# 0xPARC/plonky2-aes

Hardware: AMD Instinct MI355X
Metric: proofs/sec (AES-GCM 1 KiB circuit) (higher is better)
Workload: dtype u64 (Goldilocks field)

## Files before the change

plonky2-aes_amd/csrc/kernels.h:

```cpp
#pragma once
#include <hip/hip_runtime.h>

#include "circuit.h"
#include "witness_schedule.h"
#include "gl.h"
#include "poseidon_fast.h"
#include "poseidon_gate.h"
#include "ecstep_gate.h"
#include "zk_prf.h"

namespace p2k {
using gl::E2;
using gl::u32;
using gl::u64;

static const u64 UNSET = ~0ull;

#ifndef P2_HASH_WAVES_PER_EU
#define P2_HASH_WAVES_PER_EU 5
#endif
#define P2_HASH_WAVES __attribute__((amdgpu_waves_per_eu(P2_HASH_WAVES_PER_EU, P2_HASH_WAVES_PER_EU)))

__global__ __launch_bounds__(256) P2_HASH_WAVES void k_hash_leaves(const u64* __restrict__ data, int cols, int active_cols, size_t col_stride,
                                                      size_t batch_stride, size_t num_leaves, u64* __restrict__ digests,
                                                      size_t dig_batch_stride) {
    if ((size_t)blockIdx.x * blockDim.x + threadIdx.x >= num_leaves) return;
    const u64* d = data + (size_t)blockIdx.y * batch_stride + ((size_t)blockIdx.x * blockDim.x + threadIdx.x);
    u64 st[12];
#pragma unroll
    for (int i = 0; i < 12; i++) st[i] = 0;
    if (cols <= 4) {
        u64* out = digests + (size_t)blockIdx.y * dig_batch_stride + ((size_t)blockIdx.x * blockDim.x + threadIdx.x) * 4;
        for (int c = 0; c < 4; c++) out[c] = (c < cols && c < active_cols) ? d[(size_t)c * col_stride] : 0;
        return;
    }
    for (int c0 = 0; c0 < cols; c0 += 8) {
#pragma unroll
        for (int k = 0; k < 8; k++) {
            int c = c0 + k;
            if (c < cols) st[k] = c < active_cols ? d[(size_t)k * col_stride] : 0;
        }
        d += 8 * col_stride;
        glf::sponge_permute(st, c0, cols, active_cols);
    }
    u64* out = digests + (size_t)blockIdx.y * dig_batch_stride + ((size_t)blockIdx.x * blockDim.x + threadIdx.x) * 4;
#pragma unroll
    for (int i = 0; i < 4; i++) out[i] = st[i];
}

__global__ __launch_bounds__(256) P2_HASH_WAVES void k_hash_fri_leaves(const u64* __restrict__ vals, size_t len, size_t batch_stride, int arity,
                                                          u64* __restrict__ digests, size_t dig_batch_stride) {
    size_t leaf = (size_t)blockIdx.x * blockDim.x + threadIdx.x;
    size_t num_leaves = len / arity;
    if (leaf >= num_leaves) return;
    const u64* v = vals + (size_t)blockIdx.y * batch_stride;
    u64 st[12];
#pragma unroll
    for (int i = 0; i < 12; i++) st[i] = 0;
    int width = 2 * arity;
    for (int e0 = 0; e0 < width; e0 += 8) {
#pragma unroll
        for (int k = 0; k < 8; k++) {
            int e = e0 + k;
            if (e < width) st[k] = v[(size_t)(e & 1) * len + leaf * arity + (e >> 1)];
        }
        glf::sponge_permute(st, e0, width, width);
    }
    u64* out = digests + (size_t)blockIdx.y * dig_batch_stride + leaf * 4;
#pragma unroll
    for (int i = 0; i < 4; i++) out[i] = st[i];
}

__global__ __launch_bounds__(256) P2_HASH_WAVES void k_merkle_level(const u64* __restrict__ child, u64* __restrict__ parent, size_t num_parents,
                                                       size_t batch_stride) {
    if ((size_t)blockIdx.x * blockDim.x + threadIdx.x >= num_parents) return;
    u64 st[12];
    {
        const u64* c = child + (size_t)blockIdx.y * batch_stride + 8 * ((size_t)blockIdx.x * blockDim.x + threadIdx.x);
#pragma unroll
        for (int k = 0; k < 8; k++) st[k] = c[k];
    }
#pragma unroll
    for (int k = 8; k < 12; k++) st[k] = 0;
    glf::two_to_one_permute(st);
    u64* o = parent + (size_t)blockIdx.y * batch_stride + 4 * ((size_t)blockIdx.x * blockDim.x + threadIdx.x);
#pragma unroll
    for (int k = 0; k < 4; k++) o[k] = st[k];
}

__global__ __launch_bounds__(256) P2_HASH_WAVES void k_merkle_top(u64* __restrict__ dig, size_t batch_stride, u32 bits, u32 first_level, u32 num_levels) {
    u64* base = dig + (size_t)blockIdx.y * batch_stride;
    u32 P = ((1u << bits) >> (first_level + 1)) / gridDim.x;
    for (u32 k = 0, l = first_level; k < num_levels; k++, l++, P >>= 1) {
        if (threadIdx.x < P) {
            const size_t off_c = 4 * (((size_t)2 << bits) - ((size_t)2 << (bits - l))), off_p = 4 * (((size_t)2 << bits) - ((size_t)2 << (bits - l - 1)));
            const size_t idx = (size_t)blockIdx.x * P + threadIdx.x;
            u64 st[12];
            {
                const u64* c = base + off_c + 8 * idx;
#pragma unroll
                for (int q = 0; q < 8; q++) st[q] = c[q];
            }
#pragma unroll
            for (int q = 8; q < 12; q++) st[q] = 0;
            glf::two_to_one_permute(st);
            u64* o = base + off_p + 4 * idx;
#pragma unroll
            for (int q = 0; q < 4; q++) o[q] = st[q];
        }
        __syncthreads();
    }
}
__global__ __launch_bounds__(256) void k_merkle_top_coop(u64* __restrict__ dig, size_t batch_stride, u32 bits, u32 first_level, u32 num_levels) {
    u64* base = dig + (size_t)blockIdx.y * batch_stride;
    u32 P = ((1u << bits) >> (first_level + 1)) / gridDim.x;
    const u32 g = threadIdx.x >> 4, i = threadIdx.x & 15;
    for (u32 k = 0, l = first_level; k < num_levels; k++, l++, P >>= 1) {
        const size_t off_c = 4 * (((size_t)2 << bits) - ((size_t)2 << (bits - l))), off_p = 4 * (((size_t)2 << bits) - ((size_t)2 << (bits - l - 1)));
        for (u32 first = 0; first < P; first += blockDim.x >> 4) {
            if (first + ((threadIdx.x >> 6) << 2) < P) {
                const u32 idx = first + g;
                const bool live = idx < P;
                const size_t node = (size_t)blockIdx.x * P + (live ? idx : 0);
                u64 w = (live && i < 8) ? base[off_c + 8 * node + i] : 0;
                w = glf::poseidon_coop(w, i);
                if (live && i < 4) base[off_p + 4 * node + i] = w;
            }
        }
        __syncthreads();
    }
}

__global__ void k_poseidon_states(u64* states, size_t n) {
    size_t i = (size_t)blockIdx.x * blockDim.x + threadIdx.x;
    if (i >= n) return;
    u64 st[12];
    for (int k = 0; k < 12; k++) st[k] = states[12 * i + k];
    glf::poseidon(st);
    for (int k = 0; k < 12; k++) states[12 * i + k] = st[k];
}

__global__ __launch_bounds__(256) P2_HASH_WAVES void k_partial_rounds(u64* states, size_t n) {
    size_t i = (size_t)blockIdx.x * blockDim.x + threadIdx.x;
    if (i >= n) return;
    u64 st[12];
    for (int k = 0; k < 12; k++) st[k] = states[12 * i + k];
    glf::partial_block(st);
    for (int k = 0; k < 12; k++) states[12 * i + k] = st[k];
}

__global__ __launch_bounds__(256) P2_HASH_WAVES void k_merged_middle(u64* states, size_t n) {
    size_t i = (size_t)blockIdx.x * blockDim.x + threadIdx.x;
    if (i >= n) return;
    u64 st[12];
    for (int k = 0; k < 12; k++) st[k] = states[12 * i + k];
    glf::merged_middle(st);
    for (int k = 0; k < 12; k++) states[12 * i + k] = st[k];
}

struct NttArgs {
    const u64* in;
    u64* out;
    const u64* tw;
    const u64* pre;
    const u64* pre_tw;
    const u64* post;
    u64 post_scalar;
    size_t in_col_stride, out_col_stride, in_batch_stride, out_batch_stride;
    int logn, log_nmax, cosets;
    int bitrev_in, bitrev_out;
    int in_coset_blocks;
    u32 block_of_coset[8];
};

__global__ __launch_bounds__(1024) void k_ntt_lds(NttArgs a) {
    extern __shared__ __align__(16) u64 lds[];
    const int logn = a.logn;
    const u32 n = 1u << logn;
    const u32 col = blockIdx.x / a.cosets, coset = blockIdx.x % a.cosets;
    const u32 blk = a.block_of_coset[coset];
    const u64* in = a.in + (size_t)blockIdx.y * a.in_batch_stride + (size_t)col * a.in_col_stride + (a.in_coset_blocks ? (size_t)blk * n : 0);
    u64* out = a.out + (size_t)blockIdx.y * a.out_batch_stride + (size_t)col * a.out_col_stride + (size_t)blk * n;
    const u64* pre = a.pre ? a.pre + (size_t)coset * n : nullptr;
    const u64* post = a.post ? a.post + (size_t)coset * n : nullptr;
    for (u32 i = threadIdx.x; i < n; i += blockDim.x) {
        u64 v = in[i];
        u32 dst = a.bitrev_in ? (__brev(i) >> (32 - logn)) : i;
        if (pre) v = gl::mul_nb(v, pre[dst]);
        lds[dst] = v;
    }
    __syncthreads();
    const int tw_shift = a.log_nmax - logn;
    int s = logn - 1;
    if (logn & 1) {
        const u32 h = 1u << s;
        for (u32 t = threadIdx.x; t < (n >> 1); t += blockDim.x) {
            u32 pos = t & (h - 1);
            u32 i = ((t >> s) << (s + 1)) | pos;
            u64 x = lds[i], y = lds[i + h];
            u64 w = a.tw[(size_t)(pos << (logn - 1 - s)) << tw_shift];
            lds[i] = gl::add(x, y);
            lds[i + h] = gl::mul_nb(gl::sub(x, y), w);
        }
        __syncthreads();
        s--;
    }
    for (; s >= 1; s -= 2) {
        const u32 h = 1u << s, q = h >> 1;
        for (u32 t = threadIdx.x; t < (n >> 2); t += blockDim.x) {
            u32 pos = t & (q - 1);
            u32 i = ((t >> (s - 1)) << (s + 1)) | pos;
            u64 a0 = lds[i], a1 = lds[i + q], a2 = lds[i + h], a3 = lds[i + h + q];
            u64 w0 = a.tw[(size_t)(pos << (logn - 1 - s)) << tw_shift];
            u64 w1 = a.tw[(size_t)((pos + q) << (logn - 1 - s)) << tw_shift];
            u64 b0 = gl::add(a0, a2), b2 = gl::mul_nb(gl::sub(a0, a2), w0);
            u64 b1 = gl::add(a1, a3), b3 = gl::mul_nb(gl::sub(a1, a3), w1);
            u64 w2 = a.tw[(size_t)(pos << (logn - s)) << tw_shift];
            lds[i] = gl::add(b0, b1);
            lds[i + q] = gl::mul_nb(gl::sub(b0, b1), w2);
            lds[i + h] = gl::add(b2, b3);
            lds[i + h + q] = gl::mul_nb(gl::sub(b2, b3), w2);
        }
        __syncthreads();
    }
    for (u32 i = threadIdx.x; i < n; i += blockDim.x) {
        u32 src = a.bitrev_out ? (__brev(i) >> (32 - logn)) : i;
        u64 v = lds[src];
        if (post)
            v = gl::mul_nb(v, post[i]);
        else if (a.post_scalar != 1)
            v = gl::mul_nb(v, a.post_scalar);
        out[i] = v;
    }
}

__device__ __forceinline__ u32 ntt_pad(u32 i) { return i + (i >> 4); }
struct NttLdsWalk {
    u32 a0, step;
    __device__ __forceinline__ NttLdsWalk(u32 base, u32 stride) : a0(8 * ntt_pad(base)), step(stride >= 16 ? 8 * (stride + (stride >> 4)) : 8 * stride) {}
    __device__ __forceinline__ u64& at(u64* lds, int r) const { return *(u64*)((char*)lds + (a0 + (u32)r * step)); }
};
__device__ __forceinline__ void ntt_r16_load_tw(u64* w, const u64* __restrict__ tw, u32 tp, int m, int tw_log, int nstages) {
#pragma unroll
    for (int A = 0; A < 4; A++) {
        if (A >= nstages) break;
        const int half = 8 >> A, base = 16 - 2 * half, sh = tw_log - (m + 4 - A);
        const u32 off0 = tp << (sh + 3), dj = 1u << (m + sh + 3);
#pragma unroll
        for (int j = 0; j < 8; j++)
            if (j < half) w[base + j] = *(const u64*)((const char*)tw + (off0 + (u32)j * dj));
    }
}
template <int A>
__device__ __forceinline__ void ntt_r16_stage(u64* x, const u64* w) {
    constexpr int half = 8 >> A, base = 16 - 2 * half;
#pragma unroll
    for (int r = 0; r < 16; r++) {
        if (r & half) continue;
        const u64 u = x[r], v = x[r + half];
        x[r] = gl::add(u, v);
        x[r + half] = gl::mul_nb(gl::sub(u, v), w[base + r % half]);
    }
}
template <int A>
__device__ __forceinline__ void ntt_r16_stage_m0(u64* x, const u64* w) {
    constexpr int half = 8 >> A, base = 16 - 2 * half;
#pragma unroll
    for (int r = 0; r < 16; r++) {
        if (r & half) continue;
        const u64 u = x[r], v = x[r + half];
        x[r] = gl::add(u, v);
        x[r + half] = (r % half) ? gl::mul_nb(gl::sub(u, v), w[base + r % half]) : gl::sub(u, v);
    }
}
__device__ __forceinline__ void wave_lds_sync() {
    __builtin_amdgcn_fence(__ATOMIC_RELEASE, "wavefront");
    __builtin_amdgcn_wave_barrier();
    __builtin_amdgcn_fence(__ATOMIC_ACQUIRE, "wavefront");
}
__device__ __forceinline__ u32 xcd_swizzle(u32 b, u32 grid) { return (grid & 7) ? b : (b & 7) * (grid >> 3) + (b >> 3); }
__device__ __forceinline__ void loads_issued() { asm volatile("" ::: "memory"); }
template <bool SPLIT>
__global__ __launch_bounds__(1024) void k_ntt_r16(NttArgs a) {
    extern __shared__ __align__(16) u64 lds[];
    const int logn = SPLIT ? a.logn - 1 : a.logn;
    const u32 n = 1u << logn, T = n >> 4, t = threadIdx.x;
    const u32 bid = xcd_swizzle(blockIdx.x, gridDim.x);
    const u32 unit = SPLIT ? bid >> 1 : bid, half = SPLIT ? (bid & 1) : 0;
    const u32 col = unit / a.cosets, coset = unit % a.cosets;
    const u32 blk = a.block_of_coset[coset];
    const size_t full = (size_t)1 << a.logn;
    const u64* in = a.in + (size_t)blockIdx.y * a.in_batch_stride + (size_t)col * a.in_col_stride + (a.in_coset_blocks ? (size_t)blk * full : 0);
    u64* out = a.out + (size_t)blockIdx.y * a.out_batch_stride + (size_t)col * a.out_col_stride + (size_t)blk * full + (size_t)half * n;
    const u64* pre = a.pre ? a.pre + (size_t)coset * full : nullptr;
    const u64* post = a.post ? a.post + (size_t)coset * full : nullptr;
    u64 x[16];
    u64 w[15];
    bool tw_in_flight = false;
    if (SPLIT) {
        if (pre) {
            const u64 S = pre[n];
            const u64* scale = half ? (a.pre_tw ? a.pre_tw + (size_t)coset * n : nullptr) : pre;
            if (!half || scale) {
                u64 uu[16], vv[16], sc[16];
#pragma unroll
                for (int k = 0; k < 16; k++) uu[k] = in[t + T * k];
#pragma unroll
                for (int k = 0; k < 16; k++) vv[k] = in[t + T * k + n];
#pragma unroll
                for (int k = 0; k < 8; k++) sc[k] = scale[t + T * k];
                loads_issued();
#pragma unroll
                for (int k = 0; k < 16; k++) {
                    if (k == 4) {
                        loads_issued();
#pragma unroll
                        for (int j = 8; j < 16; j++) sc[j] = scale[t + T * j];
                        loads_issued();
                    }
                    if (k == 12) {
                        loads_issued();
                        ntt_r16_load_tw(w, a.tw, t, logn - 4, a.log_nmax, 4);
                        loads_issued();
                    }
                    const u64 v = gl::mul_nb(vv[k], S);
                    x[k] = gl::mul_nb(half ? gl::sub(uu[k], v) : gl::add(uu[k], v), sc[k]);
                }
                tw_in_flight = true;
            } else {
#pragma unroll
                for (int k = 0; k < 16; k++) {
                    const u32 i = t + T * k;
                    const u64 u = in[i], v = gl::mul_nb(in[i + n], S);
                    x[k] = gl::mul_nb(gl::mul_nb(gl::sub(u, v), pre[i]), a.tw[(size_t)i << (a.log_nmax - a.logn)]);
                }
            }
        } else {
#pragma unroll
            for (int k = 0; k < 16; k++) {
                const u32 i = t + T * k;
                const u64 u = in[i], v = in[i + n];
                x[k] = half ? gl::mul_nb(gl::sub(u, v), a.tw[(size_t)i << (a.log_nmax - a.logn)]) : gl::add(u, v);
            }
        }
    } else if (a.bitrev_in) {
#pragma unroll
        for (int k = 0; k < 16; k++) {
            const u32 i = t + T * k, dst = __brev(i) >> (32 - logn);
            u64 v = in[i];
            if (pre) v = gl::mul_nb(v, pre[dst]);
            lds[ntt_pad(dst)] = v;
        }
        __syncthreads();
        {
            const NttLdsWalk w0(t, T);
#pragma unroll
            for (int k = 0; k < 16; k++) x[k] = w0.at(lds, k);
        }
    } else {
#pragma unroll
        for (int k = 0; k < 16; k++) x[k] = in[t + T * k];
        const int rem0 = (logn & 3) ? (logn & 3) : 4;
        if (pre) {
            u64 pv[16];
#pragma unroll
            for (int k = 0; k < 16; k++) pv[k] = pre[t + T * k];
            loads_issued();
#pragma unroll
            for (int k = 0; k < 16; k++) {
                if (k == 8) {
                    loads_issued();
                    ntt_r16_load_tw(w, a.tw, t, logn - 4, a.log_nmax, rem0);
                    loads_issued();
                }
                x[k] = gl::mul_nb(x[k], pv[k]);
            }
        } else {
            ntt_r16_load_tw(w, a.tw, t, logn - 4, a.log_nmax, rem0);
            loads_issued();
        }
        tw_in_flight = true;
    }
    if (SPLIT) {
        if (!tw_in_flight) ntt_r16_load_tw(w, a.tw, t, logn - 4, a.log_nmax, 4);
        ntt_r16_stage<0>(x, w);
        ntt_r16_stage<1>(x, w);
        ntt_r16_stage<2>(x, w);
        ntt_r16_stage<3>(x, w);
        int logN = logn - 4;
        const int rem = (logN & 3) ? (logN & 3) : 4;
        int m = logN - 4;
        u32 tp = t & ((1u << m) - 1);
        ntt_r16_load_tw(w, a.tw, tp, m, a.log_nmax, rem);
        {
            const NttLdsWalk wr(t, T);
#pragma unroll
            for (int r = 0; r < 16; r++) wr.at(lds, r) = x[r];
        }
        __syncthreads();
        u32 base_idx = ((t >> m) << logN) | tp, stride = 1u << m;
        {
            const NttLdsWalk rd(base_idx, stride);
#pragma unroll
            for (int r = 0; r < 16; r++) x[r] = rd.at(lds, r);
        }
        ntt_r16_stage<0>(x, w);
        if (rem >= 2) ntt_r16_stage<1>(x, w);
        if (rem >= 3) ntt_r16_stage<2>(x, w);
        if (rem >= 4) ntt_r16_stage<3>(x, w);
        for (logN -= rem; logN >= 4; logN -= 4) {
            m = logN - 4;
            tp = t & ((1u << m) - 1);
            ntt_r16_load_tw(w, a.tw, tp, m, a.log_nmax, 4);
            {
                const NttLdsWalk wr(base_idx, stride);
#pragma unroll
                for (int r = 0; r < 16; r++) wr.at(lds, r) = x[r];
            }
            wave_lds_sync();
            base_idx = ((t >> m) << logN) | tp;
            stride = 1u << m;
            {
                const NttLdsWalk rd(base_idx, stride);
#pragma unroll
                for (int r = 0; r < 16; r++) x[r] = rd.at(lds, r);
            }
            if (m == 0) {
                ntt_r16_stage_m0<0>(x, w);
                ntt_r16_stage_m0<1>(x, w);
                ntt_r16_stage_m0<2>(x, w);
                ntt_r16_stage_m0<3>(x, w);
            } else {
                ntt_r16_stage<0>(x, w);
                ntt_r16_stage<1>(x, w);
                ntt_r16_stage<2>(x, w);
                ntt_r16_stage<3>(x, w);
            }
        }
        {
            const NttLdsWalk wr(base_idx, stride);
#pragma unroll
            for (int r = 0; r < 16; r++) wr.at(lds, r) = x[r];
        }
        wave_lds_sync();
        const u32 first = ((t >> 6) << 10) | (t & 63);
        const NttLdsWalk fin(first, 64);
#pragma unroll
        for (int k = 0; k < 16; k++) {
            u64 v = fin.at(lds, k);
            if (a.post_scalar != 1) v = gl::mul_nb(v, a.post_scalar);
            out[first + 64 * k] = v;
        }
        return;
    }
    const int rem = (logn & 3) ? (logn & 3) : 4;
    if (!tw_in_flight) ntt_r16_load_tw(w, a.tw, t, logn - 4, a.log_nmax, rem);
    ntt_r16_stage<0>(x, w);
    if (rem >= 2) ntt_r16_stage<1>(x, w);
    if (rem >= 3) ntt_r16_stage<2>(x, w);
    if (rem >= 4) ntt_r16_stage<3>(x, w);
    u32 base_idx = t, stride = T;
    for (int logN = logn - rem; logN >= 4; logN -= 4) {
        const int m = logN - 4;
        const u32 tp = t & ((1u << m) - 1);
        ntt_r16_load_tw(w, a.tw, tp, m, a.log_nmax, 4);
        {
            const NttLdsWalk wr(base_idx, stride);
#pragma unroll
            for (int r = 0; r < 16; r++) wr.at(lds, r) = x[r];
        }
        __syncthreads();
        base_idx = ((t >> m) << logN) | tp;
        stride = 1u << m;
        {
            const NttLdsWalk rd(base_idx, stride);
#pragma unroll
            for (int r = 0; r < 16; r++) x[r] = rd.at(lds, r);
        }
        if (m == 0) {
            ntt_r16_stage_m0<0>(x, w);
            ntt_r16_stage_m0<1>(x, w);
            ntt_r16_stage_m0<2>(x, w);
            ntt_r16_stage_m0<3>(x, w);
        } else {
            ntt_r16_stage<0>(x, w);
            ntt_r16_stage<1>(x, w);
            ntt_r16_stage<2>(x, w);
            ntt_r16_stage<3>(x, w);
        }
    }
    {
        const NttLdsWalk wr(base_idx, stride);
#pragma unroll
        for (int r = 0; r < 16; r++) wr.at(lds, r) = x[r];
    }
    __syncthreads();
    const NttLdsWalk fin(t, T);
#pragma unroll
    for (int k = 0; k < 16; k++) {
        const u32 i = t + T * k;
        u64 v = (!SPLIT && a.bitrev_out) ? lds[ntt_pad(__brev(i) >> (32 - logn))] : fin.at(lds, k);
        if (post)
            v = gl::mul_nb(v, post[(size_t)half * n + i]);
        else if (a.post_scalar != 1)
            v = gl::mul_nb(v, a.post_scalar);
        out[i] = v;
    }
}


struct Pass1Args {
    const u64* in;
    u64* out;
    const u64* tw;
    const u64* pre;
    const u64* out_tw;
    size_t in_col_stride, out_col_stride, in_batch_stride, out_batch_stride;
    int logn, log_n1, log_T, cosets, in_coset_blocks, xcd_swizzle;
    u32 block_of_coset[8];
};
__device__ __forceinline__ void ntt_p1_load_tw(u64* w, const u64* __restrict__ tw, u32 tp, int m, int log_T, int tw_log, int nstages) {
#pragma unroll
    for (int A = 0; A < 4; A++) {
        if (A >= nstages) break;
        const int half = 8 >> A, base = 16 - 2 * half, q = m + 4 - A - log_T;
#pragma unroll
        for (int j = 0; j < 8; j++)
            if (j < half) w[base + j] = tw[(size_t)((tp + ((u32)j << m)) >> log_T) << (tw_log - q)];
    }
}
__global__ __launch_bounds__(256, 4) void k_ntt_pass1_r16(Pass1Args a) {
    extern __shared__ __align__(16) u64 lds[];
    const u32 T = 1u << a.log_T, t = threadIdx.x;
    const int log_n2 = a.logn - a.log_n1;
    const u32 n2 = 1u << log_n2, tiles = n2 >> a.log_T;
    const u32 bid = a.xcd_swizzle ? xcd_swizzle(blockIdx.x, gridDim.x) : blockIdx.x;
    const u32 tile = bid % tiles, cc = bid / tiles, col = cc / a.cosets, coset = cc % a.cosets;
    const u32 blk = a.block_of_coset[coset];
    const size_t n = (size_t)1 << a.logn;
    const u64* in = a.in + (size_t)blockIdx.y * a.in_batch_stride + (size_t)col * a.in_col_stride + (a.in_coset_blocks ? (size_t)blk * n : 0);
    u64* out = a.out + (size_t)blockIdx.y * a.out_batch_stride + (size_t)col * a.out_col_stride + (size_t)blk * n;
    const u64* pre = a.pre ? a.pre + (size_t)coset * n : nullptr;
    const u32 j2_0 = tile << a.log_T;
    u64 x[16], w[15];
    const int rem = (a.log_n1 & 3) ? (a.log_n1 & 3) : 4;
    const u32 at = (t >> a.log_T) * n2 + j2_0 + (t & (T - 1));
    auto step = [&](int k) -> u32 { return ((256u * (u32)k) >> a.log_T) * n2 + ((256u * (u32)k) & (T - 1)); };
#pragma unroll
    for (int k = 0; k < 16; k++) x[k] = in[at + step(k)];
    if (pre) {
        u64 pv[16];
#pragma unroll
        for (int k = 0; k < 16; k++) pv[k] = pre[at + step(k)];
        loads_issued();
#pragma unroll
        for (int k = 0; k < 16; k++) {
            if (k == 8) {
                loads_issued();
                ntt_p1_load_tw(w, a.tw, t, 8, a.log_T, a.logn, rem);
                loads_issued();
            }
            x[k] = gl::mul_nb(x[k], pv[k]);
        }
    } else {
        ntt_p1_load_tw(w, a.tw, t, 8, a.log_T, a.logn, rem);
        loads_issued();
    }
    ntt_r16_stage<0>(x, w);
    if (rem >= 2) ntt_r16_stage<1>(x, w);
    if (rem >= 3) ntt_r16_stage<2>(x, w);
    if (rem >= 4) ntt_r16_stage<3>(x, w);
    u32 base_idx = t, stride = 256;
    for (int logN = 12 - rem; logN - 4 >= a.log_T; logN -= 4) {
        const int m = logN - 4;
        const u32 tp = t & ((1u << m) - 1);
        ntt_p1_load_tw(w, a.tw, tp, m, a.log_T, a.logn, 4);
#pragma unroll
        for (int r = 0; r < 16; r++) lds[ntt_pad(base_idx + (u32)r * stride)] = x[r];
        __syncthreads();
        base_idx = ((t >> m) << logN) | tp;
        stride = 1u << m;
#pragma unroll
        for (int r = 0; r < 16; r++) x[r] = lds[ntt_pad(base_idx + (u32)r * stride)];
        ntt_r16_stage<0>(x, w);
        ntt_r16_stage<1>(x, w);
        ntt_r16_stage<2>(x, w);
        ntt_r16_stage<3>(x, w);
    }
#pragma unroll
    for (int r = 0; r < 16; r++) lds[ntt_pad(base_idx + (u32)r * stride)] = x[r];
    u64 ot[16];
#pragma unroll
    for (int k = 0; k < 16; k++) ot[k] = a.out_tw[at + step(k)];
    loads_issued();
    __syncthreads();
    const NttLdsWalk fin(t, 256);
#pragma unroll
    for (int k = 0; k < 16; k++) out[at + step(k)] = gl::mul_nb(fin.at(lds, k), ot[k]);
}
__global__ void k_pass1_out_tw(const u64* __restrict__ tw, u64* __restrict__ out_tw, int logn, int log_n1) {
    const size_t i = (size_t)blockIdx.x * blockDim.x + threadIdx.x;
    if (i >> logn) return;
    const int log_n2 = logn - log_n1;
    const u32 r = (u32)(i >> log_n2), j2 = (u32)(i & (((size_t)1 << log_n2) - 1));
    const u32 k1 = log_n1 ? (__brev(r) >> (32 - log_n1)) : 0;
    out_tw[i] = tw[(size_t)k1 * j2];
}
__global__ void k_bitrev_copy(const u64* in, size_t in_col_stride, size_t in_batch_stride, u64* out, size_t out_col_stride, size_t out_batch_stride, int logn,
                              u32 blocks, const u64* post, u32 post_block_perm ) {
    const size_t n = (size_t)1 << logn;
    size_t i = (size_t)blockIdx.x * blockDim.x + threadIdx.x;
    if (i >= n) return;
    u32 col = blockIdx.z / blocks, blk = blockIdx.z % blocks;
    const u64* src = in + (size_t)blockIdx.y * in_batch_stride + (size_t)col * in_col_stride + (size_t)blk * n;
    u64* dst = out + (size_t)blockIdx.y * out_batch_stride + (size_t)col * out_col_stride + (size_t)blk * n;
    u64 v = src[__brev((u32)i) >> (32 - logn)];
    if (post) v = gl::mul(v, post[(size_t)(post_block_perm ? (__brev(blk) >> 29) : blk) * n + i]);
    dst[i] = v;
}

__global__ void k_mul_tables(u64* out, const u64* a, size_t a_stride, const u64* b, int b_shift, u32 m) {
    u32 i = blockIdx.x * blockDim.x + threadIdx.x;
    if (i >= m) return;
    out[(size_t)blockIdx.y * m + i] = gl::mul(a[(size_t)blockIdx.y * a_stride + i], b[(size_t)i << b_shift]);
}
__global__ void k_pow_table(u64* table, const u64* bases, u32 n, u64 scale) {
    u32 i = blockIdx.x * blockDim.x + threadIdx.x;
    if (i >= n) return;
    u64 b = bases[blockIdx.y];
    table[(size_t)blockIdx.y * n + i] = gl::mul(gl::pow(b, i), scale);
}

__global__ void k_quotient_chunks_rev(const u64* __restrict__ r, u64* __restrict__ t, u32 n, size_t r_batch_stride, size_t t_batch_stride,
                                  const u64* __restrict__ w8inv_pows , const u64* __restrict__ scale ) {
    u32 i = blockIdx.x * blockDim.x + threadIdx.x;
    if (i >= n) return;
    u32 ch = blockIdx.z;
    const u64* rr = r + (size_t)blockIdx.y * r_batch_stride + (size_t)ch * 8 * n + i;
    u64 v[8];
#pragma unroll
    for (int j = 0; j < 8; j++) v[j] = rr[(size_t)(__brev((u32)j) >> 29) * n];
    u64* tt = t + (size_t)blockIdx.y * t_batch_stride + (size_t)ch * 8 * n + i;
    for (int c = 0; c < 8; c++) {
        u64 acc = 0;
#pragma unroll
        for (int j = 0; j < 8; j++) acc = gl::add(acc, gl::mul(v[j], w8inv_pows[(j * c) & 7]));
        tt[(size_t)c * n] = gl::mul(acc, scale[c]);
    }
}

struct WitnessArgs {
    const p2::Op* ops;
    const p2::WLevel* levels;
    const p2::WChain* chains;
    u32 num_levels, num_slots, n_inputs;
    const u32* input_slots;
    const u64* input_values;
    u64* values;
    const u64* lut_ent;
    u32* mult;
    size_t total_lut_entries;
    int* status;
    const int32_t* wire_slot;
    u64* advice;
    u32 n, num_poseidon_rows;
};

__device__ __noinline__ int witness_poseidon_op(const WitnessArgs& a, u64* val, u32 proof, const p2::Op& o) {
    u64 w[135];
    int bad = 0;
    const u32 row = o.a;
    for (u32 c = 0; c < 12; c++) {
        w[c] = val[a.wire_slot[(size_t)c * a.n + row]];
        if (w[c] == UNSET) bad = 2;
    }
    w[p2::PG_SWAP] = val[a.wire_slot[(size_t)p2::PG_SWAP * a.n + row]];
    if (w[p2::PG_SWAP] == UNSET) bad = 2;
    if (bad) return bad;
    p2::poseidon_gate_witness(w);
    for (u32 c = p2::PG_OUT; c < 80; c++) {
        if (c == p2::PG_SWAP) continue;
        u32 sl = (u32)a.wire_slot[(size_t)c * a.n + row];
        u64 cur = val[sl];
        if (cur == UNSET)
            val[sl] = w[c];
        else if (cur != w[c])
            bad = 1;
    }
    u64* adv = a.advice + ((size_t)proof * a.num_poseidon_rows + o.aux) * 55;
    for (u32 c = 80; c < 135; c++) adv[c - 80] = w[c];
    return bad;
}

__device__ __noinline__ int witness_ecstep_op(const WitnessArgs& a, u64* val, const p2::Op& o) {
    const u32 row = o.a;
    int bad = 0;
    for (u32 c = 0; c < p2::EG_MID; c++)
        if (val[a.wire_slot[(size_t)c * a.n + row]] == UNSET) bad = 2;
    if (bad) return bad;
    p2::ecstep_row_walk([&](u32 c) { return val[a.wire_slot[(size_t)c * a.n + row]]; }, [&](u32 c, u64 v) {
        const u32 sl = (u32)a.wire_slot[(size_t)c * a.n + row];
        const u64 cur = val[sl];
        if (cur == UNSET)
            val[sl] = v;
        else if (cur != v)
            bad = 1;
    });
    return bad;
}

static const int WITNESS_KMAX = 8;
static const int WITNESS_MLP = 4;

__device__ __forceinline__ int witness_exec_chain(const WitnessArgs& a, u64* val, u32 ob, u32 cnt) {
    p2::Op o[WITNESS_KMAX];
#pragma unroll
    for (int i = 0; i < WITNESS_KMAX; i++)
        if ((u32)i < cnt) o[i] = a.ops[ob + i];
    u64 x[WITNESS_KMAX], y[WITNESS_KMAX], z[WITNESS_KMAX], cur[WITNESS_KMAX], after[WITNESS_KMAX];
#pragma unroll
    for (int i = 0; i < WITNESS_KMAX; i++) {
        x[i] = y[i] = z[i] = cur[i] = after[i] = 0;
        if ((u32)i < cnt) {
            const u32 kind = o[i].kind;
            cur[i] = val[o[i].out];
            if (kind != p2::OP_CONST) x[i] = val[o[i].a];
            if (kind != p2::OP_CONST) y[i] = val[o[i].b];
            if (kind == p2::OP_ARITH) z[i] = val[o[i].c];
        }
    }
    int worst = 0;
#pragma unroll
    for (int i = 0; i < WITNESS_KMAX; i++) {
        if ((u32)i >= cnt) break;
        const u32 kind = o[i].kind;
#pragma unroll
        for (int j = 0; j < i; j++) {
            if (o[j].out == o[i].a) x[i] = after[j];
            if (o[j].out == o[i].b) y[i] = after[j];
            if (o[j].out == o[i].c) z[i] = after[j];
            if (o[j].out == o[i].out) cur[i] = after[j];
        }
        u64 r = 0;
        int bad = 0;
        if (kind == p2::OP_ARITH) {
            if (x[i] == UNSET || y[i] == UNSET || z[i] == UNSET)
                bad = 2;
            else
                r = gl::add(gl::mul(gl::mul(x[i], y[i]), o[i].k0), gl::mul(z[i], o[i].k1));
        } else if (kind == p2::OP_CONST) {
            r = o[i].k0;
        } else if (kind == p2::OP_EQ) {
            if (x[i] == UNSET || y[i] == UNSET)
                bad = 2;
            else
                r = x[i] == y[i] ? 1 : 0;
        } else {
            bad = 2;
        }
        after[i] = cur[i];
        if (!bad) {
            if (cur[i] == UNSET) {
                val[o[i].out] = r;
                after[i] = r;
            } else if (cur[i] != r) {
                bad = 1;
            }
        }
        if (bad) worst = max(worst, bad == 1 ? 3 : 2);
    }
    return worst;
}

template <bool HAS_POSEIDON, bool CHAINS, bool HAS_EC>
__device__ __forceinline__ void witness_body(const WitnessArgs& a) {
    __shared__ int s_status;
    const u32 proof = blockIdx.x;
    u64* val = a.values + (size_t)proof * a.num_slots;
    u32* mult = a.mult + (size_t)proof * a.total_lut_entries;
    if (threadIdx.x == 0) s_status = 0;
    for (u32 i = threadIdx.x; i < a.num_slots; i += blockDim.x) val[i] = UNSET;
    __syncthreads();
    {
        const u64* iv = a.input_values + (size_t)proof * a.n_inputs;
        int bad = 0;
        for (u32 i = threadIdx.x; i < a.n_inputs; i += blockDim.x) {
            const u64 v = iv[i];
            if (v == UNSET) continue;
            if (v >= gl::P) {
                bad = 1;
                continue;
            }
            const u64 old = atomicCAS((unsigned long long*)&val[a.input_slots[i]], (unsigned long long)UNSET, (unsigned long long)v);
            if (old != UNSET && old != v) bad = 1;
        }
        if (bad) atomicMax(&s_status, 3);
    }
    __syncthreads();
    p2::Op nxt;
    bool have_nxt = false;
    p2::WLevel NL = a.levels[0];
    if (NL.single_begin + threadIdx.x < NL.single_end) {
        nxt = a.ops[NL.single_begin + threadIdx.x];
        have_nxt = true;
    }
    for (u32 lv = 0; lv < a.num_levels; lv++) {
        const p2::WLevel L = NL;
        const p2::Op first = nxt;
        const bool have_first = have_nxt;
        have_nxt = false;
        if (lv + 1 < a.num_levels) {
            NL = a.levels[lv + 1];
            if (NL.single_begin + threadIdx.x < NL.single_end) {
                nxt = a.ops[NL.single_begin + threadIdx.x];
                have_nxt = true;
            }
        }
        int worst = 0;
        if (CHAINS) {
            for (u32 ci = threadIdx.x; ci < L.chain_count; ci += blockDim.x) {
                const p2::WChain ch = a.chains[L.chain_begin + ci];
                worst = max(worst, witness_exec_chain(a, val, ch.start, min(ch.count, (u32)WITNESS_KMAX)));
            }
        }
        for (u32 k0 = L.single_begin + threadIdx.x; k0 < L.single_end; k0 += WITNESS_MLP * blockDim.x) {
            p2::Op o[WITNESS_MLP];
            bool act[WITNESS_MLP];
#pragma unroll
            for (int u = 0; u < WITNESS_MLP; u++) {
                const u32 k = k0 + u * blockDim.x;
                act[u] = k < L.single_end;
                if (act[u]) o[u] = (u == 0 && have_first && k0 == L.single_begin + threadIdx.x) ? first : a.ops[k];
            }
            u64 x[WITNESS_MLP], y[WITNESS_MLP], z[WITNESS_MLP], cur[WITNESS_MLP], ent[WITNESS_MLP];
#pragma unroll
            for (int u = 0; u < WITNESS_MLP; u++) {
                x[u] = y[u] = z[u] = cur[u] = 0;
                if (!act[u] || o[u].kind == p2::OP_POSEIDON || (HAS_EC && o[u].kind == p2::OP_ECSTEP)) continue;
                const u32 kind = o[u].kind;
                cur[u] = val[o[u].out];
                if (kind != p2::OP_CONST) x[u] = val[o[u].a];
                if (kind == p2::OP_ARITH || kind == p2::OP_EQ || kind == p2::OP_EQINV) y[u] = val[o[u].b];
                if (kind == p2::OP_ARITH) z[u] = val[o[u].c];
            }
#pragma unroll
            for (int u = 0; u < WITNESS_MLP; u++) {
                ent[u] = ~0ull;
                if (act[u] && o[u].kind == p2::OP_LOOKUP && x[u] < 65536) ent[u] = a.lut_ent[(size_t)o[u].aux * 65536 + x[u]];
            }
#pragma unroll
            for (int u = 0; u < WITNESS_MLP; u++) {
                if (!act[u]) continue;
                const u32 kind = o[u].kind;
                u64 r = 0;
                int bad = 0;
                if (kind == p2::OP_POSEIDON) {
                    if (HAS_POSEIDON) bad = witness_poseidon_op(a, val, proof, o[u]);
                    if (bad) worst = max(worst, bad == 1 ? 3 : 2);
                    continue;
                }
                if (HAS_EC && kind == p2::OP_ECSTEP) {
                    bad = witness_ecstep_op(a, val, o[u]);
                    if (bad) worst = max(worst, bad == 1 ? 3 : 2);
                    continue;
                }
                if (kind == p2::OP_ARITH) {
                    if (x[u] == UNSET || y[u] == UNSET || z[u] == UNSET)
                        bad = 2;
                    else
                        r = gl::add(gl::mul(gl::mul(x[u], y[u]), o[u].k0), gl::mul(z[u], o[u].k1));
                } else if (kind == p2::OP_CONST) {
                    r = o[u].k0;
                } else if (kind == p2::OP_LOOKUP) {
                    if (x[u] == UNSET) {
                        bad = 2;
                    } else if (ent[u] == ~0ull) {
                        bad = 1;
                    } else {
                        r = ent[u] & 0xFFFF;
                        atomicAdd(&mult[ent[u] >> 16], 1u);
                    }
                } else if (kind == p2::OP_LIMB) {
                    if (x[u] == UNSET)
                        bad = 2;
                    else
                        r = (x[u] >> o[u].k0) & ((1ull << o[u].k1) - 1);
                } else {
                    if (x[u] == UNSET || y[u] == UNSET)
                        bad = 2;
                    else if (kind == p2::OP_EQ)
                        r = x[u] == y[u] ? 1 : 0;
                    else
                        r = x[u] == y[u] ? 0 : gl::inv(gl::sub(x[u], y[u]));
                }
                if (!bad) {
                    if (cur[u] == UNSET)
                        val[o[u].out] = r;
                    else if (cur[u] != r)
                        bad = 1;
                }
                if (bad) worst = max(worst, bad == 1 ? 3 : 2);
// ... 586 lines not shown
```

Measured before the change: 771.3.

## Use scalar-base global addressing and peel final radix-16 NTT stage

```diff
diff --git a/plonky2-aes_amd/csrc/kernels.h b/plonky2-aes_amd/csrc/kernels.h
--- a/plonky2-aes_amd/csrc/kernels.h
+++ b/plonky2-aes_amd/csrc/kernels.h
@@ -237,9 +237,19 @@
 __device__ __forceinline__ u32 ntt_pad(u32 i) { return i + (i >> 4); }
 struct NttLdsWalk {
     u32 a0, step;
-    __device__ __forceinline__ NttLdsWalk(u32 base, u32 stride) : a0(8 * ntt_pad(base)), step(stride >= 16 ? 8 * (stride + (stride >> 4)) : 8 * stride) {}
+    __device__ __forceinline__ NttLdsWalk(u32 base, u32 stride) : a0(8 * ntt_pad(base)), step(stride >= 16 ? 8 * (stride + (stride >> 4)) : 8 * stride) {
+        __builtin_assume(stride == 1 || (stride & 15) == 0);
+    }
     __device__ __forceinline__ u64& at(u64* lds, int r) const { return *(u64*)((char*)lds + (a0 + (u32)r * step)); }
 };
+typedef __attribute__((address_space(1))) u64 ntt_gu64;
+__device__ __forceinline__ ntt_gu64* ntt_at(const u64* table, size_t i, u32 voff) {
+    const ntt_gu64* row = (const ntt_gu64*)(table + i);
+    asm("" : "+s"(row));
+    return (ntt_gu64*)((__attribute__((address_space(1))) char*)row + voff);
+}
+__device__ __forceinline__ u64 ntt_ld(const u64* table, size_t i, u32 voff) { return *ntt_at(table, i, voff); }
+__device__ __forceinline__ void ntt_st(u64* table, size_t i, u32 voff, u64 v) { *ntt_at(table, i, voff) = v; }
 __device__ __forceinline__ void ntt_r16_load_tw(u64* w, const u64* __restrict__ tw, u32 tp, int m, int tw_log, int nstages) {
 #pragma unroll
     for (int A = 0; A < 4; A++) {
@@ -284,10 +294,10 @@
 __global__ __launch_bounds__(1024) void k_ntt_r16(NttArgs a) {
     extern __shared__ __align__(16) u64 lds[];
     const int logn = SPLIT ? a.logn - 1 : a.logn;
-    const u32 n = 1u << logn, T = n >> 4, t = threadIdx.x;
+    const u32 n = 1u << logn, T = n >> 4, t = threadIdx.x, t8 = 8 * t;
     const u32 bid = xcd_swizzle(blockIdx.x, gridDim.x);
     const u32 unit = SPLIT ? bid >> 1 : bid, half = SPLIT ? (bid & 1) : 0;
-    const u32 col = unit / a.cosets, coset = unit % a.cosets;
+    const u32 col = __builtin_amdgcn_readfirstlane(unit / a.cosets), coset = unit - col * a.cosets;
     const u32 blk = a.block_of_coset[coset];
     const size_t full = (size_t)1 << a.logn;
     const u64* in = a.in + (size_t)blockIdx.y * a.in_batch_stride + (size_t)col * a.in_col_stride + (a.in_coset_blocks ? (size_t)blk * full : 0);
@@ -304,18 +314,18 @@
             if (!half || scale) {
                 u64 uu[16], vv[16], sc[16];
 #pragma unroll
-                for (int k = 0; k < 16; k++) uu[k] = in[t + T * k];
-#pragma unroll
-                for (int k = 0; k < 16; k++) vv[k] = in[t + T * k + n];
-#pragma unroll
-                for (int k = 0; k < 8; k++) sc[k] = scale[t + T * k];
+                for (int k = 0; k < 16; k++) uu[k] = ntt_ld(in, T * k, t8);
+#pragma unroll
+                for (int k = 0; k < 16; k++) vv[k] = ntt_ld(in, T * k + n, t8);
+#pragma unroll
+                for (int k = 0; k < 8; k++) sc[k] = ntt_ld(scale, T * k, t8);
                 loads_issued();
 #pragma unroll
                 for (int k = 0; k < 16; k++) {
                     if (k == 4) {
                         loads_issued();
 #pragma unroll
-                        for (int j = 8; j < 16; j++) sc[j] = scale[t + T * j];
+                        for (int j = 8; j < 16; j++) sc[j] = ntt_ld(scale, T * j, t8);
                         loads_issued();
                     }
                     if (k == 12) {
@@ -359,12 +369,12 @@
         }
     } else {
 #pragma unroll
-        for (int k = 0; k < 16; k++) x[k] = in[t + T * k];
+        for (int k = 0; k < 16; k++) x[k] = ntt_ld(in, T * k, t8);
         const int rem0 = (logn & 3) ? (logn & 3) : 4;
         if (pre) {
             u64 pv[16];
 #pragma unroll
-            for (int k = 0; k < 16; k++) pv[k] = pre[t + T * k];
+            for (int k = 0; k < 16; k++) pv[k] = ntt_ld(pre, T * k, t8);
             loads_issued();
 #pragma unroll
             for (int k = 0; k < 16; k++) {
@@ -408,7 +418,7 @@
         if (rem >= 2) ntt_r16_stage<1>(x, w);
         if (rem >= 3) ntt_r16_stage<2>(x, w);
         if (rem >= 4) ntt_r16_stage<3>(x, w);
-        for (logN -= rem; logN >= 4; logN -= 4) {
+        for (logN -= rem; logN >= 8; logN -= 4) {
             m = logN - 4;
             tp = t & ((1u << m) - 1);
             ntt_r16_load_tw(w, a.tw, tp, m, a.log_nmax, 4);
@@ -425,31 +435,40 @@
 #pragma unroll
                 for (int r = 0; r < 16; r++) x[r] = rd.at(lds, r);
             }
-            if (m == 0) {
-                ntt_r16_stage_m0<0>(x, w);
-                ntt_r16_stage_m0<1>(x, w);
-                ntt_r16_stage_m0<2>(x, w);
-                ntt_r16_stage_m0<3>(x, w);
-            } else {
-                ntt_r16_stage<0>(x, w);
-                ntt_r16_stage<1>(x, w);
-                ntt_r16_stage<2>(x, w);
-                ntt_r16_stage<3>(x, w);
-            }
-        }
+            ntt_r16_stage<0>(x, w);
+            ntt_r16_stage<1>(x, w);
+            ntt_r16_stage<2>(x, w);
+            ntt_r16_stage<3>(x, w);
+        }
+        ntt_r16_load_tw(w, a.tw, 0, 0, a.log_nmax, 4);
         {
             const NttLdsWalk wr(base_idx, stride);
 #pragma unroll
             for (int r = 0; r < 16; r++) wr.at(lds, r) = x[r];
+        }
+        wave_lds_sync();
+        {
+            const NttLdsWalk own(t << 4, 1);
+#pragma unroll
+            for (int r = 0; r < 16; r++) x[r] = own.at(lds, r);
+            ntt_r16_stage_m0<0>(x, w);
+            ntt_r16_stage_m0<1>(x, w);
+            ntt_r16_stage_m0<2>(x, w);
+            ntt_r16_stage_m0<3>(x, w);
+#pragma unroll
+            for (int r = 0; r < 16; r++) own.at(lds, r) = x[r];
         }
         wave_lds_sync();
         const u32 first = ((t >> 6) << 10) | (t & 63);
         const NttLdsWalk fin(first, 64);
+        ntt_gu64* const dst = ntt_at(out, 0, 8 * first);
+        ntt_gu64* dst8 = dst + 64 * 8;
+        asm("" : "+v"(dst8));
 #pragma unroll
         for (int k = 0; k < 16; k++) {
             u64 v = fin.at(lds, k);
             if (a.post_scalar != 1) v = gl::mul_nb(v, a.post_scalar);
-            out[first + 64 * k] = v;
+            (k < 8 ? dst : dst8)[64 * (k & 7)] = v;
         }
         return;
     }
@@ -460,7 +479,7 @@
     if (rem >= 3) ntt_r16_stage<2>(x, w);
     if (rem >= 4) ntt_r16_stage<3>(x, w);
     u32 base_idx = t, stride = T;
-    for (int logN = logn - rem; logN >= 4; logN -= 4) {
+    for (int logN = logn - rem; logN >= 8; logN -= 4) {
         const int m = logN - 4;
         const u32 tp = t & ((1u << m) - 1);
         ntt_r16_load_tw(w, a.tw, tp, m, a.log_nmax, 4);
@@ -477,22 +496,28 @@
 #pragma unroll
             for (int r = 0; r < 16; r++) x[r] = rd.at(lds, r);
         }
-        if (m == 0) {
-            ntt_r16_stage_m0<0>(x, w);
-            ntt_r16_stage_m0<1>(x, w);
-            ntt_r16_stage_m0<2>(x, w);
-            ntt_r16_stage_m0<3>(x, w);
-        } else {
-            ntt_r16_stage<0>(x, w);
-            ntt_r16_stage<1>(x, w);
-            ntt_r16_stage<2>(x, w);
-            ntt_r16_stage<3>(x, w);
-        }
-    }
+        ntt_r16_stage<0>(x, w);
+        ntt_r16_stage<1>(x, w);
+        ntt_r16_stage<2>(x, w);
+        ntt_r16_stage<3>(x, w);
+    }
+    ntt_r16_load_tw(w, a.tw, 0, 0, a.log_nmax, 4);
     {
         const NttLdsWalk wr(base_idx, stride);
 #pragma unroll
         for (int r = 0; r < 16; r++) wr.at(lds, r) = x[r];
+    }
+    __syncthreads();
+    {
+        const NttLdsWalk own(t << 4, 1);
+#pragma unroll
+        for (int r = 0; r < 16; r++) x[r] = own.at(lds, r);
+        ntt_r16_stage_m0<0>(x, w);
+        ntt_r16_stage_m0<1>(x, w);
+        ntt_r16_stage_m0<2>(x, w);
+        ntt_r16_stage_m0<3>(x, w);
+#pragma unroll
+        for (int r = 0; r < 16; r++) own.at(lds, r) = x[r];
     }
     __syncthreads();
     const NttLdsWalk fin(t, T);
@@ -501,10 +526,10 @@
         const u32 i = t + T * k;
         u64 v = (!SPLIT && a.bitrev_out) ? lds[ntt_pad(__brev(i) >> (32 - logn))] : fin.at(lds, k);
         if (post)
-            v = gl::mul_nb(v, post[(size_t)half * n + i]);
+            v = gl::mul_nb(v, ntt_ld(post, (size_t)half * n + T * k, t8));
         else if (a.post_scalar != 1)
             v = gl::mul_nb(v, a.post_scalar);
-        out[i] = v;
+        ntt_st(out, T * k, t8, v);
     }
 }
 
@@ -526,7 +551,7 @@
         const int half = 8 >> A, base = 16 - 2 * half, q = m + 4 - A - log_T;
 #pragma unroll
         for (int j = 0; j < 8; j++)
-            if (j < half) w[base + j] = tw[(size_t)((tp + ((u32)j << m)) >> log_T) << (tw_log - q)];
+            if (j < half) w[base + j] = ntt_ld(tw, 0, ((tp + ((u32)j << m)) >> log_T) << (tw_log - q + 3));
     }
 }
 __global__ __launch_bounds__(256, 4) void k_ntt_pass1_r16(Pass1Args a) {
@@ -544,14 +569,14 @@
     const u32 j2_0 = tile << a.log_T;
     u64 x[16], w[15];
     const int rem = (a.log_n1 & 3) ? (a.log_n1 & 3) : 4;
-    const u32 at = (t >> a.log_T) * n2 + j2_0 + (t & (T - 1));
+    const u32 at8 = 8 * ((t >> a.log_T) * n2 + j2_0 + (t & (T - 1)));
     auto step = [&](int k) -> u32 { return ((256u * (u32)k) >> a.log_T) * n2 + ((256u * (u32)k) & (T - 1)); };
 #pragma unroll
-    for (int k = 0; k < 16; k++) x[k] = in[at + step(k)];
+    for (int k = 0; k < 16; k++) x[k] = ntt_ld(in, step(k), at8);
     if (pre) {
         u64 pv[16];
 #pragma unroll
-        for (int k = 0; k < 16; k++) pv[k] = pre[at + step(k)];
+        for (int k = 0; k < 16; k++) pv[k] = ntt_ld(pre, step(k), at8);
         loads_issued();
 #pragma unroll
         for (int k = 0; k < 16; k++) {
@@ -591,12 +616,12 @@
     for (int r = 0; r < 16; r++) lds[ntt_pad(base_idx + (u32)r * stride)] = x[r];
     u64 ot[16];
 #pragma unroll
-    for (int k = 0; k < 16; k++) ot[k] = a.out_tw[at + step(k)];
+    for (int k = 0; k < 16; k++) ot[k] = ntt_ld(a.out_tw, step(k), at8);
     loads_issued();
     __syncthreads();
     const NttLdsWalk fin(t, 256);
 #pragma unroll
-    for (int k = 0; k < 16; k++) out[at + step(k)] = gl::mul_nb(fin.at(lds, k), ot[k]);
+    for (int k = 0; k < 16; k++) ntt_st(out, step(k), at8, gl::mul_nb(fin.at(lds, k), ot[k]));
 }
 __global__ void k_pass1_out_tw(const u64* __restrict__ tw, u64* __restrict__ out_tw, int logn, int log_n1) {
     const size_t i = (size_t)blockIdx.x * blockDim.x + threadIdx.x;
```

After: 771.5, median of 4. Within noise of the previous version (+0.0%).
